# PoTaTo-Mika/fish-speech

Hardware: AMD Instinct MI355X
Metric: audio-sec/wall-sec (RTF) + p50 first-sample latency, S2-Pro 4B @1/2/4/8 GPU (higher is better)
Workload: dtype bf16; 1 GPU; BASELINE config 2 per GPU: one utterance = 64-token prompt + 216 Dual-AR frames (top_k 30, top_p 0.8, temp 0.8) + codec decode [1,10,216] -> 442368 samples; global_batch=1, frames=216, prompt_len=64, first_chunk_frames=1, vocoder_chunks=first_chunk_frames, then growing 4x, vocoder=serial, parallelism=dp1

## Files before the change

### fish-speech_amd/csrc/fm_attn.hip

```cpp
#include "fm_kernels.h"
#include "fm_runtime.h"
#include "fm_attn_dev.h"
#include "fm_frag.h"
#include "fm_attn_fd_dev.h"

template <typename T>
__device__ __forceinline__ void head_prep(const T* src, int hd, bool norm, const T* nw, float eps,
                                          const float* tab, bool do_rope, float (&x0)[2],
                                          float (&x1)[2], int& np, int lane) {
    const int half = hd >> 1;
    np = 0;
    for (int p = lane; p < half; p += 64, ++np) {
        x0[np] = ld(src, 2 * p);
        x1[np] = ld(src, 2 * p + 1);
    }
    if (norm) {
        float ss = 0.f;
        for (int i = 0; i < np; ++i) ss += x0[i] * x0[i] + x1[i] * x1[i];
        ss = wave_sum(ss);
        const float rs = 1.0f / sqrtf(ss / (float)hd + eps);
        for (int i = 0; i < np; ++i) {
            const int p = lane + 64 * i;
            x0[i] = rnd<T>((x0[i] * rs) * ld(nw, 2 * p));
            x1[i] = rnd<T>((x1[i] * rs) * ld(nw, 2 * p + 1));
        }
    }
    if (do_rope) {
// ... 686 lines not shown
    }
    __syncthreads();
    if (lane == 0) {
        sh_f[wave] = best;
        sh_i[1 + wave] = bid;
    }
    __syncthreads();
    float bb = sh_f[0];
    int bi = sh_i[1];
    for (int w = 1; w < nw; ++w)
        if (cbetter(sh_f[w], sh_i[1 + w], bb, bi)) {
            bb = sh_f[w];
            bi = sh_i[1 + w];
        }
    __syncthreads();
    return bi;
}

template <typename T>
__device__ void sample_wide(const SampleArgs& a, const SlotParams& sp, int r, int slot, uint64_t* keys, int P,
                            float M, float den) {
    __shared__ int sh_i[1 + 16];
    __shared__ float sh_f[16];
    sw_sort(keys, P);
    const uint64_t step = (uint64_t)sp.step;
    int32_t* col = a.cols + (size_t)r * a.ldc;
    if (a.slow) {
        int tok = sw_draw<T>(keys, a.Nl, M, den, sp.temperature, sp.top_p, sp.top_k, sp.seed, step, 0, sh_i, sh_f);
        const int hi = sw_draw<T>(keys, a.Nl, M, den, 1.0f, 0.9f, sp.top_k, sp.seed, step, 1, sh_i, sh_f);
        if (threadIdx.x != 0) return;
        if (a.ras_enable) {
            const int32_t* prev = a.ras + (size_t)slot * a.ras_stride;
            bool inwin = false;
            for (int j = 0; j < 10; ++j) inwin |= prev[j] == tok;
            if (inwin && tok >= a.sb && tok <= a.se) tok = hi;
        }
        if (!((tok >= a.sb && tok <= a.se) || tok == a.im_end)) tok = a.im_end;
        int c = tok - a.sb;
        c = c < 0 ? 0 : (c > a.cb - 1 ? a.cb - 1 : c);
        if (sp.force) {
            tok = a.force_cols[(size_t)slot * a.ldc];
            c = a.force_cols[(size_t)slot * a.ldc + 1];
        }
        col[0] = tok;
        col[1] = c;
    } else {
        const int code = sw_draw<T>(keys, a.Nl, M, den, sp.temperature, sp.top_p, sp.top_k, sp.seed, step,
                                    (uint32_t)a.draw, sh_i, sh_f);
        if (threadIdx.x == 0)
            col[a.col_idx] = sp.force ? a.force_cols[(size_t)slot * a.ldc + a.col_idx]
                                      : ((code >= 0 && code < a.cb) ? code : 0);
    }
}

template <typename T>
__global__ __launch_bounds__(256) void sample_radix_kernel(SampleArgs a) {
    extern __shared__ __attribute__((aligned(16))) float vals[];
    __shared__ float scratch[16];
    __shared__ uint32_t hist[256];
    __shared__ uint32_t sh_prefix, sh_rem, sh_nstrict, sh_ntie;
    __shared__ float cv[64];
    __shared__ int cid[64];
    __shared__ float sv[64];
    __shared__ int sid[64];
    __shared__ int tid_[256];
    const int lane = threadIdx.x & 63, wave = threadIdx.x >> 6;
    const int r = blockIdx.x;
    const int slot = a.row_slot[r];
    const SlotParams sp = a.sp[slot];
    const float* lg = a.logits + (size_t)r * a.ldl;
    const int Nl = a.Nl;
    if (sp.force)
        for (int i = threadIdx.x; i < Nl; i += 256) a.tap[(size_t)slot * a.tap_ld + i] = lg[i];
    for (int i = threadIdx.x; i < Nl; i += 256) {
// ... 135 lines not shown
            int tok = sample_top<T>(cv, cid, K, M, den, sp.temperature, sp.top_p, sp.top_k, sp.seed, step,
                                    0, lane);
            const int hi = sample_top<T>(cv, cid, K, M, den, 1.0f, 0.9f, sp.top_k, sp.seed, step, 1, lane);
            if (a.ras_enable) {
                const int32_t* prev = a.ras + (size_t)slot * a.ras_stride;
                bool inwin = false;
                for (int j = 0; j < 10; ++j) inwin |= prev[j] == tok;
                if (inwin && tok >= a.sb && tok <= a.se) tok = hi;
            }
            if (!((tok >= a.sb && tok <= a.se) || tok == a.im_end)) tok = a.im_end;
            if (lane == 0) {
                int c = tok - a.sb;
                c = c < 0 ? 0 : (c > a.cb - 1 ? a.cb - 1 : c);
                if (sp.force) {
                    tok = a.force_cols[(size_t)slot * a.ldc];
                    c = a.force_cols[(size_t)slot * a.ldc + 1];
                }
                col[0] = tok;
                col[1] = c;
            }
        } else {
            const int code = sample_top<T>(cv, cid, K, M, den, sp.temperature, sp.top_p, sp.top_k, sp.seed,
                                           step, (uint32_t)a.draw, lane);
            if (lane == 0)
                col[a.col_idx] = sp.force ? a.force_cols[(size_t)slot * a.ldc + a.col_idx]
                                          : ((code >= 0 && code < a.cb) ? code : 0);
        }
    }
}

constexpr int SF_PER = 17;
constexpr int SF_CAP = 64;

template <int B>
__device__ __forceinline__ uint32_t sf_wave_count(uint32_t c, uint32_t* excl) {
    uint32_t tot = 0, pre = 0;
#pragma unroll
    for (int b = 0; b < B; ++b) {
        const uint64_t m = __ballot((c >> b) & 1u);
        tot += (uint32_t)__popcll(m) << b;
        if (excl) pre += (uint32_t)__builtin_amdgcn_mbcnt_hi((uint32_t)(m >> 32), __builtin_amdgcn_mbcnt_lo((uint32_t)m, 0u)) << b;
    }
    if (excl) *excl = pre;
    return tot;
}
constexpr int sf_bits(int n) { return n < 2 ? 1 : 1 + sf_bits(n >> 1); }

template <int N>
__device__ __forceinline__ uint32_t sf_radix_kth(const uint32_t (&k)[N], uint32_t K, uint32_t kmax, uint32_t cap) {
// ... 250 lines not shown
    if (a.slow) {
        int tok = sample_top<T>(cv, cid, K, M, den, sp.temperature, sp.top_p, sp.top_k, sp.seed, step, 0, lane);
        const int hi = sample_top<T>(cv, cid, K, M, den, 1.0f, 0.9f, sp.top_k, sp.seed, step, 1, lane);
        if (a.ras_enable) {
            const int32_t* prev = a.ras + (size_t)slot * a.ras_stride;
            bool inwin = false;
            for (int j = 0; j < 10; ++j) inwin |= prev[j] == tok;
            if (inwin && tok >= a.sb && tok <= a.se) tok = hi;
        }
        if (!((tok >= a.sb && tok <= a.se) || tok == a.im_end)) tok = a.im_end;
        if (lane == 0) {
            int c = tok - a.sb;
            c = c < 0 ? 0 : (c > a.cb - 1 ? a.cb - 1 : c);
            if (sp.force) {
                tok = a.force_cols[(size_t)slot * a.ldc];
                c = a.force_cols[(size_t)slot * a.ldc + 1];
            }
            col[0] = tok;
            col[1] = c;
        }
    } else {
        const int code = sample_top<T>(cv, cid, K, M, den, sp.temperature, sp.top_p, sp.top_k, sp.seed, step,
                                       (uint32_t)a.draw, lane);
        if (lane == 0)
            col[a.col_idx] = sp.force ? a.force_cols[(size_t)slot * a.ldc + a.col_idx]
                                      : ((code >= 0 && code < a.cb) ? code : 0);
    }
    record();
}

template <typename T> void launch_attn_decode2(hipStream_t s, const AttnDecArgs<T>& a, int R) {
    dim3 g1(R, a.nkv, a.maxsplit);
    static bool attr = false;
    if (!attr) {
        (void)hipFuncSetAttribute(reinterpret_cast<const void*>(&attn_decode2_kernel<T>),
                                  hipFuncAttributeMaxDynamicSharedMemorySize, 160 * 1024);
        attr = true;
    }
    attn_decode2_kernel<T><<<g1, 512, attn2_lds_bytes(a.hd, a.nh / a.nkv, a.cap, sizeof(T)), s>>>(a);
}
template <typename T, int NW, int GM> static void attn_fd_go(hipStream_t s, const AttnDecArgs<T>& a, int R) {
    const dim3 grid(R, a.nkv, a.maxsplit * FM_CEIL(a.nh / a.nkv, GM));
    switch (a.hd) {
        case 32: attn_fd_kernel<T, 32, NW, GM><<<grid, NW * 64, 0, s>>>(a); break;
        case 64: attn_fd_kernel<T, 64, NW, GM><<<grid, NW * 64, 0, s>>>(a); break;
        default: attn_fd_kernel<T, 128, NW, GM><<<grid, NW * 64, 0, s>>>(a); break;
    }
}
template <typename T, int NW> static void attn_fd_hpb(hipStream_t s, const AttnDecArgs<T>& a, int R) {
// ... 66 lines not shown
```

### fish-speech_amd/csrc/fm_kernels.h

```cpp
#pragma once
#include <algorithm>
#include "fm_common.h"
#include "fm_tune_table.h"

enum { EPI_STORE = 0, EPI_RESID = 1, EPI_SWIGLU = 2, EPI_F32 = 3 };

template <typename T> void launch_swiglu_i8(hipStream_t s, const T* t, int ldt, T* act, int lda, int inter, int R);
template <typename T> void launch_pack(hipStream_t s, const T* src, int N, int K, T* dst);
template <typename T> void launch_quant_rows(hipStream_t s, T* w, int N, int K, int8_t* q, T* scale);
template <typename T> void launch_i8_to(hipStream_t s, const int8_t* q, int64_t n, T* dst);
void launch_pack_q8(hipStream_t s, const int8_t* src, int N, int K, int8_t* dst);
void launch_pack_q8s(hipStream_t s, const int8_t* src, int N, int K, int8_t* dst);
void launch_quant4(hipStream_t s, bf16_t* w, int N, int K, int gs, uint8_t* q, uint32_t* sz);
void launch_pack_q4(hipStream_t s, const uint8_t* q, int N, int K, uint8_t* dst);
void launch_pack_q4_rows(hipStream_t s, const uint8_t* q, int N, int K, uint32_t* dst);
void launch_pack_sz4(hipStream_t s, const uint32_t* sz, int N, int K, int gs, uint32_t* dst);
void launch_pack_q4s(hipStream_t s, const uint8_t* q, int N, int K, uint32_t* dst);

template <typename T> struct LinearArgs {
    const T* W;
    const T* W2;
    const T* bias;
    const T* X;
    int ldx, R, N, K;
// ... 42 lines not shown
    float scale;
    float* part;
};

template <typename T> struct FastAttnArgs {
    const T* q;
    const int* row_slot;
    const T* kc;
    const T* vc;
    size_t slot_stride, layer_off;
    int S, nh, nkv, hd, cpos;
    float scale;
    T* out;
};

struct SlotParams {
    float temperature, top_p;
    int top_k, mask_im_end;
    uint64_t seed;
    int step;
    int force;
};

struct SampleArgs {
    const float* logits;
    int ldl, Nl;
    const int* row_slot;
    const SlotParams* sp;
    const int32_t* ras;
    int ras_stride, ras_enable;
    int slow, sb, se, im_end, cb, draw, col_idx;
    unsigned long long* dbg;
    int32_t* cols;
    int ldc;
    const int32_t* force_cols;
    float* tap;
    int tap_ld;
    int kth_fast;
};

template <typename T>
void launch_embed(hipStream_t s, const int32_t* tok, int R, const T* emb, const T* cbemb, int d,
                  int C, int cb, int sb, int se, int scale, T* x, const int* row_slot);
template <typename T>
void launch_gather_rows(hipStream_t s, const int32_t* codes, int ldc, int col, const T* table,
                        int d, int rows, int R, T* x);
template <typename T>
void launch_rmsnorm(hipStream_t s, const T* x, int ldx, const T* w, int d, float eps, T* y,
                    int ldy, int R);
template <typename T> void launch_linear(hipStream_t s, const LinearArgs<T>& a, int epi);
constexpr size_t LINEAR_PART_CAP = (size_t)8 << 20;
int linear_ksb(int N, int K, int R, int nacc, bool can_split);
template <typename T> void launch_qk_rope_cache(hipStream_t s, const QkArgs<T>& a, int R);
template <typename T>
void launch_attn(hipStream_t s, const AttnArgs<T>& a, int R, int nsplit, T* out, bool one_slot);
template <typename T> void launch_fast_attn(hipStream_t s, const FastAttnArgs<T>& a, int R);
void launch_finish(hipStream_t s, int R, const int* row_slot, int* row_pos, const int32_t* cols,
                   int ldc, int32_t* tok_in, int32_t* ras, int ras_stride, int C1, int update_ras,
                   SlotParams* sp);
template <typename T>
void launch_synth(hipStream_t s, T* dst, int64_t n, uint64_t seed, uint32_t tid, float center,
// ... 312 lines not shown
```

### fish-speech_amd/csrc/fm_llm.cpp

```cpp
#include <math.h>

#include <memory>

#include "fm_llm_model.h"

static thread_local std::string g_err;
void fm_set_error(const std::string& s) { g_err = s; }
extern "C" const char* fm_last_error(void) { return g_err.c_str(); }
extern "C" int fm_device_count(void) {
    int n = 0;
    if (hipGetDeviceCount(&n) != hipSuccess) return 0;
    return n;
}

static void check_tokens(fm_llm* m, const int32_t* tok, int T) {
    const fm_model_config& c = m->c;
    for (int t = 0; t < T; ++t) {
        const int t0 = tok[t];
        FMCHECK(t0 >= 0 && t0 < c.vocab_size, "token id out of range: " + std::to_string(t0));
        for (int q = 0; q < m->C; ++q) {
            const int v = tok[(size_t)(q + 1) * T + t];
            FMCHECK(v >= 0 && v < m->cb, "codebook token out of range: " + std::to_string(v));
        }
    }
// ... 440 lines not shown
    });
}

int fm_llm_decode_frames(fm_llm* m, const int32_t* slots, int n, int nframes, int32_t* cols) {
    return fm_guard([&] {
        FMCHECK(m && slots && cols && n >= 1 && n <= m->max_slots && nframes >= 0, "bad arguments");
        FMCHECK(m->finalized, "call fm_llm_prefill first");
        HIPCHK(hipSetDevice(m->device));
        for (int i = 0; i < n; ++i) {
            FMCHECK(slots[i] >= 0 && slots[i] < m->max_slots, "bad slot");
            for (int j = 0; j < i; ++j) FMCHECK(slots[j] != slots[i], "duplicate slot");
            FMCHECK(m->host_pos[slots[i]] + nframes <= m->c.max_seq_len, "slot would pass max_seq_len");
        }
        if (nframes == 0) return;
        const size_t per = (size_t)n * m->C1;
        if (m->h_hist_n < per * nframes) {
            if (m->h_hist) HIPCHK(hipHostFree(m->h_hist));
            m->h_hist = nullptr;
            m->h_hist_n = 0;
            HIPCHK(hipHostMalloc((void**)&m->h_hist, per * nframes * 4, hipHostMallocDefault));
            m->h_hist_n = per * nframes;
        }
        upload_frame_rows(m, slots, n);
        for (int k = 0; k < nframes; ++k) {
            launch_frame(m, n);
            HIPCHK(hipMemcpyAsync(m->h_hist + per * k, m->cols, per * 4, hipMemcpyDeviceToHost, m->stream));
        }
        chain_err_async(m);
        HIPCHK(hipStreamSynchronize(m->stream));
        chain_err_check(m);
        m->prof.collect();
        for (int i = 0; i < n; ++i) {
            m->host_pos[slots[i]] += nframes;
            m->host_step[slots[i]] += nframes;
        }
        memcpy(cols, m->h_hist, per * nframes * 4);
    });
}

static void do_generate(fm_llm* m, int slot, const int32_t* prompt, int T, int pos0, int max_new,
                        const fm_sampling* sp, int32_t* out, int* n_out) {
        FMCHECK(m && prompt && out && n_out, "null argument");
        HIPCHK(hipSetDevice(m->device));
        finalize(m);
        const fm_model_config& c = m->c;
        if (max_new <= 0 || pos0 + T + max_new > c.max_seq_len) max_new = c.max_seq_len - pos0 - T;
        FMCHECK(max_new >= 1, "prompt leaves no room to generate");
        const int C1 = m->C1;
        int32_t col[64];
        do_prefill(m, slot, prompt, T, sp, col, pos0);
        for (int q = 0; q < C1; ++q) out[(size_t)q * max_new] = col[q];
        int n = 1;
        upload_frame_rows(m, &slot, 1);
        hipEvent_t ev[2];
        HIPCHK(hipEventCreateWithFlags(&ev[0], hipEventDisableTiming));
        HIPCHK(hipEventCreateWithFlags(&ev[1], hipEventDisableTiming));
        auto issue = [&](int k) {
            launch_frame(m, 1);
            HIPCHK(hipMemcpyAsync(m->h_cols + (size_t)(k & 1) * m->max_slots * C1, m->cols, (size_t)C1 * 4,
                                  hipMemcpyDeviceToHost, m->stream));
            HIPCHK(hipEventRecord(ev[k & 1], m->stream));
        };
        const int steps = max_new - 1;
        int issued = 0;
        if (steps > 0) issue(issued++);
        for (int k = 0; k < steps; ++k) {
            if (issued < steps && issued <= k + 1) issue(issued++);
            HIPCHK(hipEventSynchronize(ev[k & 1]));
            const int32_t* hc = m->h_cols + (size_t)(k & 1) * m->max_slots * C1;
            for (int q = 0; q < C1; ++q) out[(size_t)q * max_new + n] = hc[q];
            n++;
            if (hc[0] == c.im_end_id) break;
        }
        chain_err_async(m);
        HIPCHK(hipStreamSynchronize(m->stream));
        chain_err_check(m);
        m->prof.collect();
        (void)hipEventDestroy(ev[0]);
        (void)hipEventDestroy(ev[1]);
        m->host_pos[slot] = pos0 + T + issued;
        m->host_step[slot] = 1 + issued;
// ... 92 lines not shown
```

### fish-speech_amd/csrc/fm_llm_frame.cpp

```cpp
#include <math.h>

#include <algorithm>
#include <array>

#include "fm_codec.h"
#include "fm_llm_model.h"

template <typename T> struct Run {
    typedef T type_t;
    fm_llm* m;
    hipStream_t s;
    int64_t E;
    bool rows_distinct_slots = false, bs_frame = false, x_ss = false;
    struct BsPending {
        bool on = false;
        const float* slab = nullptr;
        int kparts = 0, d = 0, R = 0;
        void* res = nullptr;
        void* out = nullptr;
        const void* sc = nullptr;
    } pend;
    std::vector<std::array<int, 2>> segs;
    void set_pending(const float* slab, int kparts, int d, int R, void* res, void* out, const void* sc) {
        pend = BsPending{true, slab, kparts, d, R, res, out, sc};
// ... 1135 lines not shown
            const SmallPath p0 = small_path(c0, false), p1 = small_path(c1, false);
            if (!(p0.kv0 && p1.fw && p1.rf && !p1.att_wo && (l == 0 ? p1.tab : p1.row_here))) return false;
        }
        return true;
    }
    void fast_pair(const void* hidden) {
        const fm_model_config& c = m->c;
        const KsbPlan kp = plan(m->fdm, 1);
        const int nl = m->fdm.n_layer;
        for (int l = 0; l < nl; ++l)
            block_small(m->fdm, m->fast[l], 1, l == 0, hidden, c.fast_dim, m->cols, 1, m->fx, m->fh, true, 1, l, kp, m->fx,
                        false, l == nl - 1 ? 2 : 1, m->femb);
        fast_head(1, (const char*)m->fx + (size_t)c.fast_dim * sizeof(T));
    }
    int fast_open(int n, const void* hidden) {
        if (fast_pair_live(n)) {
            fast_pair(hidden);
            return 2;
        }
        fast_small(n, 0, false, hidden);
        return 1;
    }

    void frame_tail_small(int n, bool ras_enable, bool sample, const void* hidden) {
        if (sample) {
            SampleArgs a = sargs(true, ras_enable, 0);
            run_("sample", 0, 0, [&] { launch_sample_radix<T>(s, a, n); });
        }
        int cc = fast_open(n, hidden);
        if (cc == 2 && sample) {
            SampleArgs a = sargs(false, 0, 1);
            run_("sample", 0, 0, [&] { launch_sample_radix<T>(s, a, n); });
        }
        for (; cc < m->C; ++cc) {
            fast_small(n, cc, true, hidden);
            if (sample) {
                SampleArgs a = sargs(false, 0, cc);
                run_("sample", 0, 0, [&] { launch_sample_radix<T>(s, a, n); });
            }
        }
    }

    void decode_frame_small(int n) {
        run_("other", 0, 0, [&] {
            launch_embed<T>(s, m->tok_in, n, (const T*)m->emb, (const T*)m->cbemb, m->c.dim, m->C, m->cb,
                            m->c.semantic_begin_id, m->c.semantic_end_id, m->c.scale_codebook_embeddings,
                            (T*)m->x, m->frame_slot);
        });
        slow_small(n);
        const KsbPlan kp = plan(m->sd, n);
        const void* hid = head_small(nullptr, true, n, kp.w2);
        frame_tail_small(n, true, true, hid);
        chain_flush();
        launch_finish(s, n, m->frame_slot, m->frame_pos, m->cols, m->C1, m->tok_in, m->ras, m->C1 * 10, m->C1,
                      1, m->sp);
    }

    void slow_layers(int R, const int* rslot, const int* rpos) {
        x_ss = false;
        for (int l = 0; l < m->sd.n_layer; ++l)
            block(m->sd, m->slow[l], R, rslot, rpos, -1, false, m->kc, m->vc, m->slot_stride,
                  (size_t)l * m->layer_stride, m->S, m->rope, m->x, m->h, m->xn);
        flush();
    }

    void head_and_hidden(const void* xlast, int n) {
        const fm_model_config& c = m->c;
        chain_flush();
        run_("norm", 0, 0, [&] {
            launch_rmsnorm<T>(s, (const T*)xlast, c.dim, (const T*)m->norm, c.dim, c.norm_eps, (T*)m->xnl,
                              c.dim, n);
        });
        linear(m->head_c, nullptr, m->xnl, c.dim, n, m->Nhead, c.dim, nullptr, m->Nhead,
               nullptr, 0, m->logits, EPI_F32, "linear");
        const void* src = c.norm_fastlayer_input ? m->xnl : xlast;
        if (m->fproj_w)
            linear(m->fproj_w, m->fproj_b, src, c.dim, n, c.fast_dim, c.dim, m->fx, c.fast_dim,
                   nullptr, 0, nullptr, EPI_STORE, "linear");
// ... 43 lines not shown
        a.tap = slow ? m->tap_slow : m->tap_fast + (size_t)(c - 1) * m->cb;
        a.tap_ld = slow ? m->Nhead : (m->C - 1) * m->cb;
        return a;
    }

    void frame_tail(int n, bool ras_enable, bool sample) {
        if (sample) {
            SampleArgs a = sargs(true, ras_enable, 0);
            run_("sample", 0, 0, [&] { launch_sample_radix<T>(s, a, n); });
        }
        fast_pass(n, 0, false);
        for (int cc = 1; cc < m->C; ++cc) {
            run_("other", 0, 0, [&] {
                launch_gather_rows<T>(s, m->cols, m->C1, cc, (const T*)m->femb, m->c.fast_dim, m->cb, n, (T*)m->fx);
            });
            fast_pass(n, cc, true);
            if (sample) {
                SampleArgs a = sargs(false, 0, cc);
                run_("sample", 0, 0, [&] { launch_sample_radix<T>(s, a, n); });
            }
        }
    }

    void decode_frame(int n) {
        if (n <= GEMV_MAX_ROWS) {
            decode_frame_small(n);
            return;
        }
        run_("other", 0, 0, [&] {
            launch_embed<T>(s, m->tok_in, n, (const T*)m->emb, (const T*)m->cbemb, m->c.dim, m->C, m->cb,
                            m->c.semantic_begin_id, m->c.semantic_end_id, m->c.scale_codebook_embeddings,
                            (T*)m->x, m->frame_slot);
        });
        rows_distinct_slots = true;
        bs_frame = true;
        slow_layers(n, m->frame_slot, m->frame_pos);
        rows_distinct_slots = false;
        head_and_hidden(m->x, n);
        frame_tail(n, true, true);
        bs_frame = false;
        chain_flush();
        launch_finish(s, n, m->frame_slot, m->frame_pos, m->cols, m->C1, m->tok_in, m->ras, m->C1 * 10,
                      m->C1, 1, m->sp);
    }

    const void* prefill_slow(int slot, const int32_t* tokens, int Tn, int pos0) {
        const int C1 = m->C1;
        std::vector<int32_t> rows((size_t)PREFILL_CHUNK * C1);
        std::vector<int> rs(PREFILL_CHUNK, slot), rp(PREFILL_CHUNK);
// ... 96 lines not shown
    const bool prof_on = m->prof.on;
    t.dbg = nullptr;
    m->prof.on = false;
    try {
        Run<bf16_t> r(m);
        const GemvArgs<bf16_t> a = r.qkv_args(d, m->fast[0], 1);
        for (int code = 0; code < m->cb; ++code)
            r.qkv_first(d, m->fast[0], a, 1, m->femb, m->c.fast_dim, m->qkv0_iota, code,
                        (bf16_t*)m->qkv0 + (size_t)code * d.nqkv(), false);
        r.chain_flush();
        HIPCHK(hipGetLastError());
        HIPCHK(hipStreamSynchronize(m->stream));
    } catch (...) {
        t.dbg = dbg;
        m->prof.on = prof_on;
        throw;
    }
    t.dbg = dbg;
    m->prof.on = prof_on;
    m->qkv0_epoch = t.epoch;
    m->qkv0_built = true;
}

void launch_frame(fm_llm* m, int n) {
    ensure_qkv0(m);
    if (m->use_graph && !m->prof.on) {
        auto it = m->graphs.find(n);
        if (it == m->graphs.end()) {
            hipGraph_t g;
            HIPCHK(hipStreamBeginCapture(m->stream, hipStreamCaptureModeThreadLocal));
            with_prec(m, [&](auto& r) { r.decode_frame(n); });
            HIPCHK(hipStreamEndCapture(m->stream, &g));
            hipGraphExec_t ge;
            HIPCHK(hipGraphInstantiate(&ge, g, nullptr, nullptr, 0));
            HIPCHK(hipGraphDestroy(g));
            it = m->graphs.emplace(n, ge).first;
        }
        HIPCHK(hipGraphLaunch(it->second, m->stream));
    } else {
        with_prec(m, [&](auto& r) { r.decode_frame(n); });
    }
}

void decode_frame_eager(fm_llm* m, int n) {
    with_prec(m, [&](auto& r) { r.decode_frame(n); });
}

void prefill_frame(fm_llm* m, int slot, const int32_t* tokens, int T, int pos0) {
    ensure_qkv0(m);
    with_prec(m, [&](auto& r) {
        const void* last = r.prefill_slow(slot, tokens, T, pos0);
        const void* hid = r.head_small(last, false, 1, 1);
        r.frame_tail_small(1, false, true, hid);
    });
}

void prefill_batch_frame(fm_llm* m, int n, const int32_t* slots, const int32_t* const* toks, const int32_t* T,
                         const int32_t* pos0) {
    ensure_qkv0(m);
    with_prec(m, [&](auto& r) {
        r.prefill_multi(n, slots, toks, T, pos0);
        if (n <= GEMV_MAX_ROWS) {
            const void* hid = r.head_small(m->plast, false, n, 1);
// ... 46 lines not shown
```

### fish-speech_amd/csrc/fm_llm_kernels.hip

```cpp
#include "fm_kernels.h"
#include "fm_runtime.h"
#include "fm_frag.h"

template <typename T>
__global__ __launch_bounds__(256) void embed_kernel(const int32_t* __restrict__ tok, int R,
                                                    const T* __restrict__ emb,
                                                    const T* __restrict__ cbemb, int d, int C,
                                                    int cb, int sb, int se, int scale,
                                                    T* __restrict__ x,
                                                    const int* __restrict__ row_slot) {
    const int r = blockIdx.x;
    if (r >= R) return;
    const int32_t* t = tok + (size_t)(row_slot ? row_slot[r] : r) * (C + 1);
    const int i = 8 * (blockIdx.y * 256 + threadIdx.x);
    if (i >= d) return;
    int t0 = t[0];
    t0 = t0 < 0 ? 0 : t0;
    if (row_slot) t0 = t0 > se ? se : t0;
    const bool sem = t0 >= sb && t0 <= se;
    float v[8] = {0.f, 0.f, 0.f, 0.f, 0.f, 0.f, 0.f, 0.f};
    if (sem) {
        for (int q = 0; q < C; ++q) {
            float c8[8];
            int cq = t[1 + q];
            cq = cq < 0 ? 0 : (cq >= cb ? cb - 1 : cq);
            load8(cbemb + (size_t)(cq + q * cb) * d + i, c8);
#pragma unroll
            for (int u = 0; u < 8; ++u) v[u] += c8[u];
        }
    }
    float e8[8];
    load8(emb + (size_t)t0 * d + i, e8);
    const float inv = sqrtf((float)(C + 1));
#pragma unroll
    for (int u = 0; u < 8; ++u) {
        float e = rnd<T>(e8[u] + (sem ? rnd<T>(v[u]) : 0.f));
        if (scale && sem) e = rnd<T>(e / inv);
        st(x, (size_t)r * d + i + u, e);
    }
}

template <typename T>
__global__ __launch_bounds__(256) void gather_rows_kernel(const int32_t* __restrict__ codes,
                                                          int ldc, int col, const T* __restrict__ table,
                                                          int d, int rows, T* __restrict__ x) {
    const int r = blockIdx.x;
    int c = codes[(size_t)r * ldc + col];
    c = c < 0 ? 0 : (c >= rows ? rows - 1 : c);
    for (int i = threadIdx.x; i < d; i += blockDim.x) x[(size_t)r * d + i] = table[(size_t)c * d + i];
}

constexpr int RN_MAXC = 8;
template <typename T>
__global__ __launch_bounds__(256) void rmsnorm_wave_kernel(const T* __restrict__ x, int ldx,
                                                           const T* __restrict__ w, int d, float eps,
                                                           T* __restrict__ y, int ldy, int R) {
    const int lane = threadIdx.x & 63;
    const int r = blockIdx.x * 4 + (threadIdx.x >> 6);
    if (r >= R) return;
    const T* xr = x + (size_t)r * ldx;
    float v[RN_MAXC][8];
    float ss = 0.f;
// ... 944 lines not shown
```

### fish-speech_amd/csrc/fm_llm_model.h

```cpp
#pragma once
#include <hip/hip_runtime.h>

#include <algorithm>

#include "fm_kernels.h"
#include "fm_runtime.h"

static constexpr int PREFILL_CHUNK = 1024;
static constexpr int ATTN_PIECE = 256;
static constexpr int ATTN_SPLIT = 64;
static constexpr int GEMV_MAX_ROWS = 8;
static constexpr int KSB_MAX = 8;

inline int attn2_frame_cap(int hd, int g, size_t esz, bool batched) {
    const int cap = attn2_cap(hd, g, esz), knob = batched ? fm_tuning().attn_cap_batched : fm_tuning().attn_cap;
    return knob ? std::min(cap, knob) : cap;
}
struct AttnSlowPlan {
    int kernel, nwb, cap;
    int hpb = 4;
};
inline int fd_hpb_rows(int R) { return R <= GEMV_MAX_ROWS ? fm_tuning().fd_hpb : 4; }
inline AttnSlowPlan attn_slow_plan(int R, int hd, int g, int cap0) {
    const FmTuning& tu = fm_tuning();
// ... 93 lines not shown
    unsigned* chain_cnt = nullptr;
    int* chain_err = nullptr;
    int* h_chain_err = nullptr;
    void* plast = nullptr;
    float *part = nullptr, *logits = nullptr, *flogits = nullptr;
    void* act2 = nullptr;
    int* attn_cnt = nullptr;
    float *ssX = nullptr, *ssH = nullptr;
    int* tickets = nullptr;
    float* skpart = nullptr;
    long long skpart_cap = 0;
    float *slabA = nullptr, *slabB = nullptr;
    float *bsA = nullptr, *bsB = nullptr;
    float* bsQ = nullptr;
    int *frame_slot = nullptr, *frame_pos = nullptr, *prow_slot = nullptr, *prow_pos = nullptr;
    int32_t *tok_in = nullptr, *cols = nullptr, *ptok = nullptr, *ras = nullptr;
    SlotParams* sp = nullptr;
    int32_t* force_cols = nullptr;
    float *tap_slow = nullptr, *tap_fast = nullptr;
    std::vector<int> host_force;
    int32_t* h_cols = nullptr;
    int32_t* h_hist = nullptr;
    size_t h_hist_n = 0;
    std::vector<int> host_pos, host_step;
    std::vector<int> uploaded_slots;
    bool use_graph = true;
    std::map<int, hipGraphExec_t> graphs;
    Profiler prof;
    std::vector<void*> allocs;
    int quant = FM_QUANT_NONE;
    int q4_gs = 0;
    int qmode() const { return quant == FM_QUANT_INT8 ? 1 : (quant == FM_QUANT_INT4 ? 2 : 0); }
    int* fin_cnt = nullptr;
    float* fin_ss = nullptr;
    bool compact = false;
    bool streams_codes() const { return quant != FM_QUANT_INT4 || fm_tuning().int4_stream || compact; }
    int64_t mem[7] = {0, 0, 0, 0, 0, 0, 0};
    int mem_cat = 6;
    bool row_ok = false;
    bool row_qkv_ok = false;
    bool row_w13_ok = false;
    uint32_t* fxt = nullptr;
    uint32_t* sxt = nullptr;
    int32_t* fiota = nullptr;
    void* qkv0 = nullptr;
    int32_t* qkv0_iota = nullptr;
// ... 2 lines not shown
    struct Prefix {
        void* buf = nullptr;
        int npos = 0;
        size_t bytes = 0;
    };
    std::map<int, Prefix> prefixes;
    int next_prefix_id = 1;
    int* pfx_slots = nullptr;

    ~fm_llm() {
        if (device >= 0) (void)hipSetDevice(device);
        for (auto& g : graphs) (void)hipGraphExecDestroy(g.second);
        for (auto& kv : w) {
            if (kv.second.p) (void)hipFree(kv.second.p);
            if (kv.second.q) (void)hipFree(kv.second.q);
        }
        for (void* p : allocs) (void)hipFree(p);
        for (auto& kv : prefixes) (void)hipFree(kv.second.buf);
        if (h_cols) (void)hipHostFree(h_cols);
        if (h_hist) (void)hipHostFree(h_hist);
        if (h_chain_err) (void)hipHostFree(h_chain_err);
        if (stream) (void)hipStreamDestroy(stream);
    }
    void* dalloc(size_t bytes, bool zero = true) {
        void* p = nullptr;
        if (bytes == 0) bytes = 16;
        hipError_t e = hipMalloc(&p, bytes);
        if (e != hipSuccess)
            throw FmError{FM_ERR_OOM, "hipMalloc(" + std::to_string(bytes) + ") failed: " + hipGetErrorString(e)};
        if (zero) HIPCHK(hipMemsetAsync(p, 0, bytes, stream));
        allocs.push_back(p);
        mem[mem_cat] += (int64_t)bytes;
        return p;
    }
};

void add_t(fm_llm* m, const std::string& n, int64_t rows, int64_t cols);
void build_inventory(fm_llm* m);
DTensor& tensor_for(fm_llm* m, const char* name, int64_t numel);
bool is_quant_linear(const std::string& n);
std::string base_of(const std::string& n);
void finalize(fm_llm* m);
void ensure_qkv0(fm_llm* m);
void launch_frame(fm_llm* m, int n);
void decode_frame_eager(fm_llm* m, int n);
void prefill_frame(fm_llm* m, int slot, const int32_t* tokens, int T, int pos0);
void prefill_batch_frame(fm_llm* m, int n, const int32_t* slots, const int32_t* const* toks, const int32_t* T,
                         const int32_t* pos0);
void teacher_frame(fm_llm* m, int slot, const int32_t* x, int S, int pos0, const int32_t* next_col, float* lg,
                   float* hidden, float* fast_logits);
```

### fish-speech_amd/csrc/fm_llm_weights.cpp

```cpp
#include "fm_llm_model.h"

void add_t(fm_llm* m, const std::string& n, int64_t rows, int64_t cols) {
    DTensor t;
    t.rows = rows;
    t.cols = cols;
    t.numel = rows * cols;
    m->w[n] = t;
}
static void add_stack(fm_llm* m, const std::string& pre, const StackDims& s) {
    for (int i = 0; i < s.n_layer; ++i) {
        std::string p = pre + std::to_string(i) + ".";
        add_t(m, p + "attention.wqkv.weight", s.nqkv(), s.dim);
        if (s.qkv_bias) add_t(m, p + "attention.wqkv.bias", 1, s.nqkv());
        add_t(m, p + "attention.wo.weight", s.dim, s.nq());
        if (s.o_bias) add_t(m, p + "attention.wo.bias", 1, s.dim);
        if (s.qk_norm) {
            add_t(m, p + "attention.q_norm.weight", 1, s.hd);
            add_t(m, p + "attention.k_norm.weight", 1, s.hd);
        }
        add_t(m, p + "feed_forward.w1.weight", s.inter, s.dim);
        add_t(m, p + "feed_forward.w3.weight", s.inter, s.dim);
        add_t(m, p + "feed_forward.w2.weight", s.dim, s.inter);
        add_t(m, p + "ffn_norm.weight", 1, s.dim);
        add_t(m, p + "attention_norm.weight", 1, s.dim);
// ... 459 lines not shown
        m->skpart_cap = 16ll << 20;
        m->skpart = (float*)m->dalloc((size_t)m->skpart_cap * sizeof(float), false);
    }
    HIPCHK(hipMemsetAsync(m->attn_cnt, 0, ncnt * sizeof(int), m->stream));
    m->slabA = (float*)m->dalloc((size_t)KSB_MAX * std::min(n, GEMV_MAX_ROWS) * dmax * 4);
    m->slabB = (float*)m->dalloc((size_t)KSB_MAX * std::min(n, GEMV_MAX_ROWS) * dmax * 4);
    if (n > GEMV_MAX_ROWS) {
        m->bsA = (float*)m->dalloc((size_t)BS_KPARTS * 32 * dmax * 4, false);
        m->bsB = (float*)m->dalloc((size_t)BS_KPARTS * 32 * dmax * 4, false);
        m->bsQ = (float*)m->dalloc((size_t)BS_KPARTS * 32 * std::max(m->sd.nqkv(), m->fdm.nqkv()) * 4, false);
    }
    m->logits = (float*)m->dalloc((size_t)n * m->Nhead * 4);
    m->flogits = (float*)m->dalloc((size_t)n * m->cb * 4);
    m->frame_slot = (int*)m->dalloc(n * 4);
    m->frame_pos = (int*)m->dalloc(n * 4);
    m->prow_slot = (int*)m->dalloc(PREFILL_CHUNK * 4);
    m->prow_pos = (int*)m->dalloc(PREFILL_CHUNK * 4);
    m->pfx_slots = (int*)m->dalloc((size_t)n * 4);
    m->tok_in = (int32_t*)m->dalloc((size_t)n * m->C1 * 4);
    m->cols = (int32_t*)m->dalloc((size_t)n * m->C1 * 4);
    m->ptok = (int32_t*)m->dalloc((size_t)PREFILL_CHUNK * m->C1 * 4);
    m->ras = (int32_t*)m->dalloc((size_t)n * m->C1 * 10 * 4);
    m->sp = (SlotParams*)m->dalloc(sizeof(SlotParams) * n);
    m->force_cols = (int32_t*)m->dalloc((size_t)n * m->C1 * 4);
    m->tap_slow = (float*)m->dalloc((size_t)n * m->Nhead * 4);
    m->tap_fast = (float*)m->dalloc((size_t)n * std::max(m->C - 1, 1) * m->cb * 4);
    m->host_force.assign(n, 0);
    HIPCHK(hipHostMalloc((void**)&m->h_cols, (size_t)2 * n * m->C1 * 4, hipHostMallocDefault));
    m->host_pos.assign(n, 0);
    m->host_step.assign(n, 0);
    HIPCHK(hipStreamSynchronize(m->stream));
    m->finalized = true;
}
```

### fish-speech_amd/csrc/fm_tune_table.h

```cpp
#ifndef FM_TUNE_RULES
#define FM_TUNE_RULES
enum { FM_RULE_BOOL, FM_RULE_ANY, FM_RULE_SET, FM_RULE_RANGE, FM_RULE_MULT16 };
template <typename... V> constexpr int fm_knob_set(V... v) { return (0 | ... | (1 << v)); }
#define FM_BOOL FM_RULE_BOOL, 0, 0
#define FM_ANY FM_RULE_ANY, 0, 0
#define FM_SET(...) FM_RULE_SET, fm_knob_set(__VA_ARGS__), 0
#define FM_RANGE(lo, hi) FM_RULE_RANGE, lo, hi
#define FM_MIN(lo) FM_RULE_RANGE, lo, 0x7fffffff
#define FM_MULT16 FM_RULE_MULT16, 0, 0
#define FM_ZERO_OR_MULT16 FM_RULE_MULT16, 1, 0
#endif

#ifdef FM_KNOB
FM_KNOB(gemv_nt, 1, FM_BOOL)
FM_KNOB(gemv_u, 8, FM_SET(2, 4, 8))
FM_KNOB(gemv_wpb, 4, FM_SET(4, 8))
FM_KNOB(sampler_kth, 1, FM_BOOL)
FM_KNOB(sampler_fast, 1, FM_BOOL)
FM_KNOB(attn_cap, 32, FM_ZERO_OR_MULT16)
FM_KNOB(attn_wo, 0, FM_BOOL)
FM_KNOB(ksb_blocks, 512, FM_MIN(1))
FM_KNOB(batched_fused_attn, 1, FM_BOOL)
FM_KNOB(attn_cap_batched, 128, FM_ZERO_OR_MULT16)
FM_KNOB(linear_u32, 4, FM_SET(4, 8))
// ... 50 lines not shown
FM_KNOB(q_u, 4, FM_SET(2, 4, 8, 16))
FM_KNOB(fin8, 1, FM_BOOL)
FM_KNOB(fin_split, 0, FM_RANGE(0, 16))
FM_KNOB(bstream_q8, 1, FM_BOOL)
FM_KNOB(bstream_q4, 1, FM_BOOL)
FM_KNOB(int4_stream, 1, FM_BOOL)
FM_KNOB(fw_delay, 0, FM_RANGE(0, 1000))
FM_KNOB(fw_cheap, 0, FM_BOOL)
FM_KNOB(fw_prio, 0, FM_BOOL)
FM_KNOB(fattn_wo, 1, FM_BOOL)
FM_KNOB(fattn_ilp, 1, FM_BOOL)
FM_KNOB(row_qkv_rp, 8, FM_SET(4, 8, 16))
FM_KNOB(rowgemv_q4, 31, FM_RANGE(0, 31))
FM_KNOB(rowgemv, 123, FM_RANGE(0, 127))
FM_KNOB(row_copies, 1, FM_BOOL)
FM_KNOB(prefix_vec, 1, FM_BOOL)
FM_KNOB(fast_pair, 1, FM_BOOL)
FM_KNOB(fast_dead_q, 1, FM_RANGE(0, 3))
FM_KNOB(slow_attn_wo, 2, FM_RANGE(0, 2))
FM_KNOB(slow_aw_delay, 40, FM_RANGE(0, 300))
FM_KNOB(slow_aw_sleep, 1, FM_SET(1, 4, 16))
FM_KNOB(slow_aw_cheap, 1, FM_BOOL)
FM_KNOB(slow_attn_wo_q, 0, FM_RANGE(0, 2))
#endif
```

Measured before the change: 12.62 audio-sec/wall-sec.

## Fuse frame finish, history capture and next embed into last sampler

Adds a frame-edge epilogue to the final fast-codebook sampling kernel. It can perform the finish step (token window shift, position and step increment), record per-frame codes into a device history buffer, and compute the next frame's embedding in place. This removes the separate finish and embed launches and the per-frame device-to-host copy of codes, which cuts launch and copy overhead on the serial decode path. Only the finish bit is enabled by default. The cost is extra work in the sampler tail and more graph variants keyed by edge bits.

```diff
diff --git a/fish-speech_amd/csrc/fm_attn.hip b/fish-speech_amd/csrc/fm_attn.hip
--- a/fish-speech_amd/csrc/fm_attn.hip
+++ b/fish-speech_amd/csrc/fm_attn.hip
@@ -3,6 +3,7 @@
 #include "fm_attn_dev.h"
 #include "fm_frag.h"
 #include "fm_attn_fd_dev.h"
+#include "fm_frame_edge.h"
 
 template <typename T>
 __device__ __forceinline__ void head_prep(const T* src, int hd, bool norm, const T* nw, float eps,
@@ -735,6 +736,7 @@
                             float M, float den) {
     __shared__ int sh_i[1 + 16];
     __shared__ float sh_f[16];
+    __shared__ int32_t edge_tk[64];
     sw_sort(keys, P);
     const uint64_t step = (uint64_t)sp.step;
     int32_t* col = a.cols + (size_t)r * a.ldc;
@@ -760,9 +762,9 @@
     } else {
         const int code = sw_draw<T>(keys, a.Nl, M, den, sp.temperature, sp.top_p, sp.top_k, sp.seed, step,
                                     (uint32_t)a.draw, sh_i, sh_f);
-        if (threadIdx.x == 0)
-            col[a.col_idx] = sp.force ? a.force_cols[(size_t)slot * a.ldc + a.col_idx]
-                                      : ((code >= 0 && code < a.cb) ? code : 0);
+        const int val = sp.force ? a.force_cols[(size_t)slot * a.ldc + a.col_idx] : ((code >= 0 && code < a.cb) ? code : 0);
+        if (threadIdx.x == 0) col[a.col_idx] = val;
+        if (a.edge.bits && threadIdx.x < 64) frame_edge_row<T, 1>(a, r, slot, val, (int)threadIdx.x, edge_tk);
     }
 }
 
@@ -944,9 +946,9 @@
         } else {
             const int code = sample_top<T>(cv, cid, K, M, den, sp.temperature, sp.top_p, sp.top_k, sp.seed,
                                            step, (uint32_t)a.draw, lane);
-            if (lane == 0)
-                col[a.col_idx] = sp.force ? a.force_cols[(size_t)slot * a.ldc + a.col_idx]
-                                          : ((code >= 0 && code < a.cb) ? code : 0);
+            const int val = sp.force ? a.force_cols[(size_t)slot * a.ldc + a.col_idx] : ((code >= 0 && code < a.cb) ? code : 0);
+            if (lane == 0) col[a.col_idx] = val;
+            if (a.edge.bits) frame_edge_row<T, 1>(a, r, slot, val, lane, tid_);
         }
     }
 }
@@ -1243,9 +1245,9 @@
     } else {
         const int code = sample_top<T>(cv, cid, K, M, den, sp.temperature, sp.top_p, sp.top_k, sp.seed, step,
                                        (uint32_t)a.draw, lane);
-        if (lane == 0)
-            col[a.col_idx] = sp.force ? a.force_cols[(size_t)slot * a.ldc + a.col_idx]
-                                      : ((code >= 0 && code < a.cb) ? code : 0);
+        const int val = sp.force ? a.force_cols[(size_t)slot * a.ldc + a.col_idx] : ((code >= 0 && code < a.cb) ? code : 0);
+        if (lane == 0) col[a.col_idx] = val;
+        if (a.edge.bits) frame_edge_row<T, sizeof(T) == 2 ? 12 : 1>(a, r, slot, val, lane, cid);
     }
     record();
 }
diff --git a/fish-speech_amd/csrc/fm_frame_edge.h b/fish-speech_amd/csrc/fm_frame_edge.h
--- /dev/null
+++ b/fish-speech_amd/csrc/fm_frame_edge.h
@@ -0,0 +1,80 @@
+#pragma once
+#include "fm_common.h"
+#include "fm_kernels.h"
+
+template <typename T, int QB = 1>
+__device__ __forceinline__ void embed_row8(const int32_t* t, bool decode, const T* __restrict__ emb,
+                                           const T* __restrict__ cbemb, int d, int C, int cb, int sb, int se,
+                                           int scale, T* __restrict__ x, int r, int i) {
+    int t0 = t[0];
+    t0 = t0 < 0 ? 0 : t0;
+    if (decode) t0 = t0 > se ? se : t0;
+    const bool sem = t0 >= sb && t0 <= se;
+    float v[8] = {0.f, 0.f, 0.f, 0.f, 0.f, 0.f, 0.f, 0.f};
+    float e8[8];
+    if constexpr (QB > 1) load8(emb + (size_t)t0 * d + i, e8);
+    if (sem) {
+        for (int q0 = 0; q0 < C; q0 += QB) {
+            float c8[QB][8];
+#pragma unroll
+            for (int j = 0; j < QB; ++j) {
+                const int q = q0 + j < C ? q0 + j : C - 1;
+                int cq = t[1 + q];
+                cq = cq < 0 ? 0 : (cq >= cb ? cb - 1 : cq);
+                load8(cbemb + (size_t)(cq + q * cb) * d + i, c8[j]);
+            }
+#pragma unroll
+            for (int j = 0; j < QB; ++j)
+                if (q0 + j < C) {
+#pragma unroll
+                    for (int u = 0; u < 8; ++u) v[u] += c8[j][u];
+                }
+        }
+    }
+    if constexpr (QB == 1) load8(emb + (size_t)t0 * d + i, e8);
+    const float inv = sqrtf((float)(C + 1));
+#pragma unroll
+    for (int u = 0; u < 8; ++u) {
+        float e = rnd<T>(e8[u] + (sem ? rnd<T>(v[u]) : 0.f));
+        if (scale && sem) e = rnd<T>(e / inv);
+        st(x, (size_t)r * d + i + u, e);
+    }
+}
+
+__device__ __forceinline__ void frame_finish_row(const FrameEdgeArgs& e, int r, int slot, int32_t cq, int lane) {
+    if (lane < e.C1) {
+        e.tok_in[(size_t)slot * e.C1 + lane] = cq;
+        int32_t* w = e.ras + (size_t)slot * (e.C1 * 10) + lane * 10;
+        int32_t keep[9];
+#pragma unroll
+        for (int j = 0; j < 9; ++j) keep[j] = w[j + 1];
+#pragma unroll
+        for (int j = 0; j < 9; ++j) w[j] = keep[j];
+        w[9] = cq;
+    }
+    if (lane == 0) {
+        e.row_pos[r] += 1;
+        e.sp[slot].step += 1;
+    }
+}
+
+template <typename T, int QB>
+__device__ __forceinline__ void frame_edge_row(const SampleArgs& a, int r, int slot, int32_t last, int lane,
+                                               int32_t* tk) {
+    const FrameEdgeArgs& e = a.edge;
+    const int32_t* col = a.cols + (size_t)r * a.ldc;
+    int32_t cq = 0;
+    if (lane < e.C1) cq = lane == a.col_idx ? last : col[lane];
+    const int k = (e.bits & FRAME_EDGE_HIST) ? e.hist_k[r] : 0;
+    if (e.bits & FRAME_EDGE_FINISH) frame_finish_row(e, r, slot, cq, lane);
+    if (e.bits & FRAME_EDGE_HIST) {
+        if (k < e.hist_cap && lane < e.C1) e.hist[((size_t)k * gridDim.x + r) * e.C1 + lane] = cq;
+        if (lane == 0) e.hist_k[r] = k + 1;
+    }
+    if (e.bits & FRAME_EDGE_EMBED) {
+        if (lane < e.C1) tk[lane] = cq;
+        __builtin_amdgcn_wave_barrier();
+        for (int i = 8 * lane; i < e.d; i += 8 * 64)
+            embed_row8<T, QB>(tk, true, (const T*)e.emb, (const T*)e.cbemb, e.d, e.C, e.cb, a.sb, a.se, e.scale, (T*)e.x, r, i);
+    }
+}
diff --git a/fish-speech_amd/csrc/fm_kernels.h b/fish-speech_amd/csrc/fm_kernels.h
--- a/fish-speech_amd/csrc/fm_kernels.h
+++ b/fish-speech_amd/csrc/fm_kernels.h
@@ -88,6 +88,22 @@
     int force;
 };
 
+enum { FRAME_EDGE_FINISH = 1, FRAME_EDGE_HIST = 2, FRAME_EDGE_EMBED = 4 };
+struct FrameEdgeArgs {
+    int bits, C1;
+    int* row_pos;
+    int32_t* tok_in;
+    int32_t* ras;
+    SlotParams* sp;
+    int32_t* hist;
+    int* hist_k;
+    int hist_cap;
+    const void* emb;
+    const void* cbemb;
+    void* x;
+    int d, C, cb, scale;
+};
+
 struct SampleArgs {
     const float* logits;
     int ldl, Nl;
@@ -103,6 +119,7 @@
     float* tap;
     int tap_ld;
     int kth_fast;
+    FrameEdgeArgs edge;
 };
 
 template <typename T>
diff --git a/fish-speech_amd/csrc/fm_llm.cpp b/fish-speech_amd/csrc/fm_llm.cpp
--- a/fish-speech_amd/csrc/fm_llm.cpp
+++ b/fish-speech_amd/csrc/fm_llm.cpp
@@ -486,10 +486,15 @@
             m->h_hist_n = per * nframes;
         }
         upload_frame_rows(m, slots, n);
+        const bool dev_hist = (frame_edge_bits(m, n) & FRAME_EDGE_HIST) != 0;
+        if (dev_hist) HIPCHK(hipMemsetAsync(m->d_hist_k, 0, (size_t)n * sizeof(int), m->stream));
         for (int k = 0; k < nframes; ++k) {
-            launch_frame(m, n);
-            HIPCHK(hipMemcpyAsync(m->h_hist + per * k, m->cols, per * 4, hipMemcpyDeviceToHost, m->stream));
-        }
+            launch_frame(m, n, k > 0);
+            if (!dev_hist)
+                HIPCHK(hipMemcpyAsync(m->h_hist + per * k, m->cols, per * 4, hipMemcpyDeviceToHost, m->stream));
+        }
+        if (dev_hist)
+            HIPCHK(hipMemcpyAsync(m->h_hist, m->d_hist, per * nframes * 4, hipMemcpyDeviceToHost, m->stream));
         chain_err_async(m);
         HIPCHK(hipStreamSynchronize(m->stream));
         chain_err_check(m);
@@ -520,7 +525,7 @@
         HIPCHK(hipEventCreateWithFlags(&ev[0], hipEventDisableTiming));
         HIPCHK(hipEventCreateWithFlags(&ev[1], hipEventDisableTiming));
         auto issue = [&](int k) {
-            launch_frame(m, 1);
+            launch_frame(m, 1, k > 0);
             HIPCHK(hipMemcpyAsync(m->h_cols + (size_t)(k & 1) * m->max_slots * C1, m->cols, (size_t)C1 * 4,
                                   hipMemcpyDeviceToHost, m->stream));
             HIPCHK(hipEventRecord(ev[k & 1], m->stream));
diff --git a/fish-speech_amd/csrc/fm_llm_frame.cpp b/fish-speech_amd/csrc/fm_llm_frame.cpp
--- a/fish-speech_amd/csrc/fm_llm_frame.cpp
+++ b/fish-speech_amd/csrc/fm_llm_frame.cpp
@@ -1181,38 +1181,60 @@
         return 1;
     }
 
-    void frame_tail_small(int n, bool ras_enable, bool sample, const void* hidden) {
+    FrameEdgeArgs edge_args(int bits) const {
+        FrameEdgeArgs e{};
+        e.bits = bits;
+        e.C1 = m->C1;
+        e.row_pos = m->frame_pos;
+        e.tok_in = m->tok_in;
+        e.ras = m->ras;
+        e.sp = m->sp;
+        e.hist = m->d_hist;
+        e.hist_k = m->d_hist_k;
+        e.hist_cap = m->c.max_seq_len;
+        e.emb = m->emb;
+        e.cbemb = m->cbemb;
+        e.x = m->x;
+        e.d = m->c.dim;
+        e.C = m->C;
+        e.cb = m->cb;
+        e.scale = m->c.scale_codebook_embeddings;
+        return e;
+    }
+    void frame_tail_small(int n, bool ras_enable, bool sample, const void* hidden, int edge = 0) {
+        auto fast_sample = [&](int c) {
+            SampleArgs a = sargs(false, 0, c);
+            if (edge && c == m->C - 1) a.edge = edge_args(edge);
+            run_("sample", 0, 0, [&] { launch_sample_radix<T>(s, a, n); });
+        };
         if (sample) {
             SampleArgs a = sargs(true, ras_enable, 0);
             run_("sample", 0, 0, [&] { launch_sample_radix<T>(s, a, n); });
         }
         int cc = fast_open(n, hidden);
-        if (cc == 2 && sample) {
-            SampleArgs a = sargs(false, 0, 1);
-            run_("sample", 0, 0, [&] { launch_sample_radix<T>(s, a, n); });
-        }
+        if (cc == 2 && sample) fast_sample(1);
         for (; cc < m->C; ++cc) {
             fast_small(n, cc, true, hidden);
-            if (sample) {
-                SampleArgs a = sargs(false, 0, cc);
-                run_("sample", 0, 0, [&] { launch_sample_radix<T>(s, a, n); });
-            }
-        }
-    }
-
-    void decode_frame_small(int n) {
-        run_("other", 0, 0, [&] {
-            launch_embed<T>(s, m->tok_in, n, (const T*)m->emb, (const T*)m->cbemb, m->c.dim, m->C, m->cb,
-                            m->c.semantic_begin_id, m->c.semantic_end_id, m->c.scale_codebook_embeddings,
-                            (T*)m->x, m->frame_slot);
-        });
+            if (sample) fast_sample(cc);
+        }
+    }
+
+    void decode_frame_small(int n, bool steady) {
+        const int edge = frame_edge_bits(m, n);
+        if (!(steady && (edge & FRAME_EDGE_EMBED)))
+            run_("other", 0, 0, [&] {
+                launch_embed<T>(s, m->tok_in, n, (const T*)m->emb, (const T*)m->cbemb, m->c.dim, m->C, m->cb,
+                                m->c.semantic_begin_id, m->c.semantic_end_id, m->c.scale_codebook_embeddings,
+                                (T*)m->x, m->frame_slot);
+            });
         slow_small(n);
         const KsbPlan kp = plan(m->sd, n);
         const void* hid = head_small(nullptr, true, n, kp.w2);
-        frame_tail_small(n, true, true, hid);
+        frame_tail_small(n, true, true, hid, edge);
         chain_flush();
-        launch_finish(s, n, m->frame_slot, m->frame_pos, m->cols, m->C1, m->tok_in, m->ras, m->C1 * 10, m->C1,
-                      1, m->sp);
+        if (!(edge & FRAME_EDGE_FINISH))
+            launch_finish(s, n, m->frame_slot, m->frame_pos, m->cols, m->C1, m->tok_in, m->ras, m->C1 * 10, m->C1,
+                          1, m->sp);
     }
 
     void slow_layers(int R, const int* rslot, const int* rpos) {
@@ -1302,9 +1324,9 @@
         }
     }
 
-    void decode_frame(int n) {
+    void decode_frame(int n, bool steady = false) {
         if (n <= GEMV_MAX_ROWS) {
-            decode_frame_small(n);
+            decode_frame_small(n, steady);
             return;
         }
         run_("other", 0, 0, [&] {
@@ -1447,23 +1469,26 @@
     m->qkv0_built = true;
 }
 
-void launch_frame(fm_llm* m, int n) {
+void launch_frame(fm_llm* m, int n, bool steady) {
     ensure_qkv0(m);
+    const int edge = frame_edge_bits(m, n);
+    steady = steady && (edge & FRAME_EDGE_EMBED);
     if (m->use_graph && !m->prof.on) {
-        auto it = m->graphs.find(n);
+        const int key = n + 8192 * (2 * edge + (steady ? 1 : 0));
+        auto it = m->graphs.find(key);
         if (it == m->graphs.end()) {
             hipGraph_t g;
             HIPCHK(hipStreamBeginCapture(m->stream, hipStreamCaptureModeThreadLocal));
-            with_prec(m, [&](auto& r) { r.decode_frame(n); });
+            with_prec(m, [&](auto& r) { r.decode_frame(n, steady); });
             HIPCHK(hipStreamEndCapture(m->stream, &g));
             hipGraphExec_t ge;
             HIPCHK(hipGraphInstantiate(&ge, g, nullptr, nullptr, 0));
             HIPCHK(hipGraphDestroy(g));
-            it = m->graphs.emplace(n, ge).first;
+            it = m->graphs.emplace(key, ge).first;
         }
         HIPCHK(hipGraphLaunch(it->second, m->stream));
     } else {
-        with_prec(m, [&](auto& r) { r.decode_frame(n); });
+        with_prec(m, [&](auto& r) { r.decode_frame(n, steady); });
     }
 }
 
diff --git a/fish-speech_amd/csrc/fm_llm_kernels.hip b/fish-speech_amd/csrc/fm_llm_kernels.hip
--- a/fish-speech_amd/csrc/fm_llm_kernels.hip
+++ b/fish-speech_amd/csrc/fm_llm_kernels.hip
@@ -1,6 +1,7 @@
 #include "fm_kernels.h"
 #include "fm_runtime.h"
 #include "fm_frag.h"
+#include "fm_frame_edge.h"
 
 template <typename T>
 __global__ __launch_bounds__(256) void embed_kernel(const int32_t* __restrict__ tok, int R,
@@ -14,30 +15,7 @@
     const int32_t* t = tok + (size_t)(row_slot ? row_slot[r] : r) * (C + 1);
     const int i = 8 * (blockIdx.y * 256 + threadIdx.x);
     if (i >= d) return;
-    int t0 = t[0];
-    t0 = t0 < 0 ? 0 : t0;
-    if (row_slot) t0 = t0 > se ? se : t0;
-    const bool sem = t0 >= sb && t0 <= se;
-    float v[8] = {0.f, 0.f, 0.f, 0.f, 0.f, 0.f, 0.f, 0.f};
-    if (sem) {
-        for (int q = 0; q < C; ++q) {
-            float c8[8];
-            int cq = t[1 + q];
-            cq = cq < 0 ? 0 : (cq >= cb ? cb - 1 : cq);
-            load8(cbemb + (size_t)(cq + q * cb) * d + i, c8);
-#pragma unroll
-            for (int u = 0; u < 8; ++u) v[u] += c8[u];
-        }
-    }
-    float e8[8];
-    load8(emb + (size_t)t0 * d + i, e8);
-    const float inv = sqrtf((float)(C + 1));
-#pragma unroll
-    for (int u = 0; u < 8; ++u) {
-        float e = rnd<T>(e8[u] + (sem ? rnd<T>(v[u]) : 0.f));
-        if (scale && sem) e = rnd<T>(e / inv);
-        st(x, (size_t)r * d + i + u, e);
-    }
+    embed_row8<T>(t, row_slot != nullptr, emb, cbemb, d, C, cb, sb, se, scale, x, r, i);
 }
 
 template <typename T>
diff --git a/fish-speech_amd/csrc/fm_llm_model.h b/fish-speech_amd/csrc/fm_llm_model.h
--- a/fish-speech_amd/csrc/fm_llm_model.h
+++ b/fish-speech_amd/csrc/fm_llm_model.h
@@ -139,6 +139,8 @@
     int32_t* h_cols = nullptr;
     int32_t* h_hist = nullptr;
     size_t h_hist_n = 0;
+    int32_t* d_hist = nullptr;
+    int* d_hist_k = nullptr;
     std::vector<int> host_pos, host_step;
     std::vector<int> uploaded_slots;
     bool use_graph = true;
@@ -187,7 +189,7 @@
         if (h_chain_err) (void)hipHostFree(h_chain_err);
         if (stream) (void)hipStreamDestroy(stream);
     }
-    void* dalloc(size_t bytes, bool zero = true) {
+    void* dalloc(size_t bytes, bool zero = true, bool book = true) {
         void* p = nullptr;
         if (bytes == 0) bytes = 16;
         hipError_t e = hipMalloc(&p, bytes);
@@ -195,7 +197,7 @@
             throw FmError{FM_ERR_OOM, "hipMalloc(" + std::to_string(bytes) + ") failed: " + hipGetErrorString(e)};
         if (zero) HIPCHK(hipMemsetAsync(p, 0, bytes, stream));
         allocs.push_back(p);
-        mem[mem_cat] += (int64_t)bytes;
+        if (book) mem[mem_cat] += (int64_t)bytes;
         return p;
     }
 };
@@ -207,8 +209,12 @@
 std::string base_of(const std::string& n);
 void finalize(fm_llm* m);
 void ensure_qkv0(fm_llm* m);
-void launch_frame(fm_llm* m, int n);
+void launch_frame(fm_llm* m, int n, bool steady = false);
 void decode_frame_eager(fm_llm* m, int n);
+inline int frame_edge_bits(const fm_llm* m, int n) {
+    if (n > GEMV_MAX_ROWS || m->C < 2 || m->C1 > 64 || !m->d_hist) return 0;
+    return fm_tuning().frame_edge & (FRAME_EDGE_FINISH | FRAME_EDGE_HIST | FRAME_EDGE_EMBED);
+}
 void prefill_frame(fm_llm* m, int slot, const int32_t* tokens, int T, int pos0);
 void prefill_batch_frame(fm_llm* m, int n, const int32_t* slots, const int32_t* const* toks, const int32_t* T,
                          const int32_t* pos0);
diff --git a/fish-speech_amd/csrc/fm_llm_weights.cpp b/fish-speech_amd/csrc/fm_llm_weights.cpp
--- a/fish-speech_amd/csrc/fm_llm_weights.cpp
+++ b/fish-speech_amd/csrc/fm_llm_weights.cpp
@@ -505,6 +505,8 @@
     m->ptok = (int32_t*)m->dalloc((size_t)PREFILL_CHUNK * m->C1 * 4);
     m->ras = (int32_t*)m->dalloc((size_t)n * m->C1 * 10 * 4);
     m->sp = (SlotParams*)m->dalloc(sizeof(SlotParams) * n);
+    m->d_hist = (int32_t*)m->dalloc((size_t)m->c.max_seq_len * std::min(n, GEMV_MAX_ROWS) * m->C1 * 4, false, false);
+    m->d_hist_k = (int*)m->dalloc((size_t)GEMV_MAX_ROWS * sizeof(int), true, false);
     m->force_cols = (int32_t*)m->dalloc((size_t)n * m->C1 * 4);
     m->tap_slow = (float*)m->dalloc((size_t)n * m->Nhead * 4);
     m->tap_fast = (float*)m->dalloc((size_t)n * std::max(m->C - 1, 1) * m->cb * 4);
diff --git a/fish-speech_amd/csrc/fm_tune_table.h b/fish-speech_amd/csrc/fm_tune_table.h
--- a/fish-speech_amd/csrc/fm_tune_table.h
+++ b/fish-speech_amd/csrc/fm_tune_table.h
@@ -96,4 +96,5 @@
 FM_KNOB(slow_aw_sleep, 1, FM_SET(1, 4, 16))
 FM_KNOB(slow_aw_cheap, 1, FM_BOOL)
 FM_KNOB(slow_attn_wo_q, 0, FM_RANGE(0, 2))
+FM_KNOB(frame_edge, 1, FM_RANGE(0, 7))
 #endif
```

New measurement: 12.62 audio-sec/wall-sec. Within noise of the previous version (-0.0%).
